# leotimus/recommender-tensorflow

Hardware: AMD Instinct MI355X
Metric: examples/sec DeepFM batch=65536 (full train step) (higher is better)
Workload: dtype f32 (MLP GEMM operands: fp16 hi+lo split, 3 products, fp32 accumulate)

## Files before the change

### __graft_entry__.py

```python
import os
import subprocess
import sys

ROOT = os.path.dirname(os.path.abspath(__file__))
PKG = os.path.join(ROOT, "recommender-tensorflow_amd")
for _p in (ROOT, PKG):
    if _p not in sys.path:
        sys.path.insert(0, _p)


def build():
    csrc = os.path.join(PKG, "csrc")
    subprocess.run(["make", "-C", csrc, "-j", str(min(8, os.cpu_count() or 1))], check=True)
    from mi355x_rec import _lib
    lib = _lib.load()
    print("built:", lib.mi_build_info().decode(), "->", _lib.LIB_PATH)
    import oracle


def smoke():
    import numpy as np
    import torch
    from mi355x_rec.engine import DeepFM, OptimizerSpec
    from oracle import deepfm as O, optimizers as OO
    from oracle.columns import ml100k_fields, sorted_fields

    assert torch.cuda.is_available(), "smoke() needs a GPU"
    cases = (([f[4] for f in sorted_fields(ml100k_fields())], 4, [16, 16], 32),
             ([40 + 3 * i for i in range(26)], 64, [512, 256, 128], 64))
    for vocab, E, hidden, B in cases:
        rng = np.random.default_rng(0)
        p = O.init_params(rng, vocab, E, hidden, dtype=np.float32, lin_scale=0.01)
        m = DeepFM(vocab, embedding_size=E, hidden_units=hidden, optimizer=OptimizerSpec("Adam", 0.001), device="cuda:0")
        m.load_oracle_params(p)
        st = O.TrainState(p, OO.Hyper("Adam", 0.001))
        for _ in range(3):
            ids = np.stack([rng.integers(0, v, B) for v in vocab], 1).astype(np.int32)
            y = (rng.random(B) < 0.3).astype(np.uint8)
            lo, logit_o = O.train_step(p, st, ids, y)
            lg, logit_g = m.train_step(torch.from_numpy(ids).cuda(), torch.from_numpy(y).cuda())
            err = float(np.max(np.abs(logit_g.cpu().numpy() - logit_o)) / (np.sqrt(np.mean(logit_o ** 2)) + 1e-30))
            assert abs(lg.item() - float(lo)) / abs(float(lo)) < 2e-5 and err < 5e-5, (E, lg.item(), float(lo), err)
        print("smoke ok (E=%d, hidden %s, planes path: %s): loss %.6f (oracle %.6f), logits err %.2e" % (
            E, hidden, bool(m.planes), lg.item(), float(lo), err))


if __name__ == "__main__":
    build()
    if "--smoke" in sys.argv:
        smoke()
```

### recommender-tensorflow_amd/csrc/optim.hip

```cpp
#include "common.h"
#include "optim_rules.h"
#include <algorithm>

namespace {

constexpr int kBlock = 256;

__global__ __launch_bounds__(kBlock) void dense_apply_k(float* __restrict__ w, float* __restrict__ s0,
                                                        float* __restrict__ s1,
                                                        const float* __restrict__ g, int64_t n,
                                                        Hp h, const mi_step_state_t* __restrict__ st) {
  if (st) h.lr_t = st->lr_t;
  const int64_t stride = static_cast<int64_t>(gridDim.x) * kBlock;
  for (int64_t i = static_cast<int64_t>(blockIdx.x) * kBlock + threadIdx.x; i < n; i += stride) {
    float wv = w[i], a = s0 ? s0[i] : 0.f, b = s1 ? s1[i] : 0.f;
    dense_rule(h, wv, a, b, g[i]);
    w[i] = wv;
    if (s0) s0[i] = a;
    if (s1) s1[i] = b;
  }
}

typedef float f32x4_t __attribute__((ext_vector_type(4)));
__device__ __forceinline__ float4 ld4_nt(const float* p) {
// ... 198 lines not shown
        if constexpr (STORE) store_row(a, uu, l, lane_on, g, gl);
        else apply_row(a, h, r, l, lane_on, w, g, gl, load_row_state(a, h, r, l, lane_on));
      }
      __syncthreads();
    }
  }
}

__device__ __forceinline__ float sqrt_rn_fixup(float x) {
  float s = __builtin_amdgcn_sqrtf(x);
  const float sm = __uint_as_float(__float_as_uint(s) - 1u), sp = __uint_as_float(__float_as_uint(s) + 1u);
  const float rm = fmaf(-sm, s, x), rp = fmaf(-sp, s, x);
  s = (rm <= 0.f) ? sm : s;
  s = (rp > 0.f) ? sp : s;
  return s;
}
__device__ __forceinline__ float sqrt_rn_inrange(float x) {
  const float r = __builtin_amdgcn_rsqf(x);
  float s = x * r, h = 0.5f * r;
  const float e = fmaf(-h, s, 0.5f);
  h = fmaf(h, e, h);
  s = fmaf(s, e, s);
  const float d = fmaf(-s, s, x);
  return fmaf(d, h, s);
}
__device__ __forceinline__ float div_rn_inrange(float n, float d) {
  float r = __builtin_amdgcn_rcpf(d);
  const float e = fmaf(-d, r, 1.0f);
  r = fmaf(e, r, r);
  float q = n * r;
  const float e2 = fmaf(-d, q, n);
  q = fmaf(e2, r, q);
  const float e3 = fmaf(-d, q, n);
  return fmaf(e3, r, q);
}
__device__ __forceinline__ bool catchup_in_range(float m, float v) {
  const float am = fabsf(m);
  return (am == 0.f || (am >= 0x1p-50f && am <= 0x1p60f)) && v >= 0x1p-93f && v <= 0x1p20f;
}
__device__ __forceinline__ bool catchup_params_in_range(int steps, float lr_last, float eps, float b1, float b2) {
  return steps <= 200 && lr_last >= 0x1p-17f && eps >= 0x1p-40f && eps <= 1.f &&
         b1 >= 0.9f && b1 <= 1.f && b2 >= 0.99f && b2 <= 1.f;
}

struct RhoSplit { float hi, lo; };
__device__ __forceinline__ RhoSplit rho_split(float b2) {
  const double r = sqrt(static_cast<double>(b2));
  RhoSplit q;
  q.hi = static_cast<float>(r);
  q.lo = static_cast<float>(r - static_cast<double>(q.hi));
  return q;
}
__device__ __forceinline__ float bounded_step(float w, float u, float s0, float rj, float eps) {
  return fmaf(-u, __builtin_amdgcn_rcpf(fmaf(s0, rj, eps)), w);
}

__global__ __launch_bounds__(kBlock) void catchup_lin_k(
    float* __restrict__ lin_w, float* __restrict__ lm, float* __restrict__ lv, const int32_t* __restrict__ last_step,
    const int32_t* __restrict__ uniq_rows, const int32_t* __restrict__ num_uniq, int64_t n_max, int step_to,
    const float* __restrict__ lr_table, float b1, float b2, float eps, bool defer_slots, int st,
    const mi_step_state_t* __restrict__ ss, bool bounded) {
  if (ss) step_to = ss->step - 1;
  const int64_t u = static_cast<int64_t>(blockIdx.x) * kBlock + threadIdx.x;
  const int64_t count = uniq_rows ? static_cast<int64_t>(*num_uniq) : n_max;
  const bool on = u < count;
  const int64_t r = (on ? (uniq_rows ? static_cast<int64_t>(uniq_rows[u]) : u) : 0) * st;
  const int ls = on ? last_step[r] : step_to;
  const bool work = on && ls > 0 && ls < step_to;
  float w = 0.f, m = 0.f, v = 0.f;
  if (work) { w = lin_w[r]; m = lm[r]; v = lv[r]; }
  if (bounded) {
    if (work) {
      const RhoSplit rho = rho_split(b2);
      const float s0 = sqrtf(v);
      float rj = 1.f;
      for (int s = ls + 1; s <= step_to; ++s) {
        rj = fmaf(rj, rho.lo, rj * rho.hi);
        m = m * b1;
        w = bounded_step(w, lr_table[s] * m, s0, rj, eps);
      }
      if (!defer_slots)
        for (int s = ls + 1; s <= step_to; ++s) v = v * b2;
      lin_w[r] = w;
      if (!defer_slots) { lm[r] = m; lv[r] = v; }
    }
    return;
  }
  const bool ok = !work || (catchup_params_in_range(step_to - ls, lr_table[step_to], eps, b1, b2) && catchup_in_range(m, v));
  if (__ballot(!ok) == 0) {
    if (work)
      for (int s = ls + 1; s <= step_to; ++s) {
        m = m * b1; v = v * b2;
        w = w - div_rn_inrange(lr_table[s] * m, sqrt_rn_inrange(v) + eps);
      }
  } else if (work) {
    replay(w, m, v, ls + 1, step_to, lr_table, b1, b2, eps);
  }
  if (work) {
    lin_w[r] = w;
    if (!defer_slots) { lm[r] = m; lv[r] = v; }
  }
}

template <int LPR>
__global__ __launch_bounds__(kBlock) void sparse_catchup_k(
    float* __restrict__ table, float* __restrict__ tm, float* __restrict__ tv,
    int32_t* __restrict__ last_step, const int32_t* __restrict__ uniq_rows,
    const int32_t* __restrict__ num_uniq, int64_t n_max, int E, int step_to,
    const float* __restrict__ lr_table, float b1, float b2, float eps, bool defer_slots, int st,
    const mi_step_state_t* __restrict__ ss, bool keep_stamps, int64_t ts) {
  if (ss) step_to = ss->step - 1;
  const int64_t u = (static_cast<int64_t>(blockIdx.x) * kBlock + threadIdx.x) / LPR;
  const int l = threadIdx.x & (LPR - 1);
  const int64_t count = uniq_rows ? static_cast<int64_t>(*num_uniq) : n_max;
  if (u >= count) return;
  const int64_t r = uniq_rows ? static_cast<int64_t>(uniq_rows[u]) : u;
  const int ls = last_step[r * st];
  if (ls >= step_to) return;
  if (ls > 0) {
    if (table && 4 * l < E) {
      const int64_t o = r * ts + 4 * l;
      float4 w = ld4(table + o), m = ld4_nt(tm + o), v = ld4_nt(tv + o);
      const bool ok = catchup_params_in_range(step_to - ls, lr_table[step_to], eps, b1, b2) && catchup_in_range(m.x, v.x) &&
                      catchup_in_range(m.y, v.y) && catchup_in_range(m.z, v.z) && catchup_in_range(m.w, v.w);
      if (__ballot(!ok) == 0) {
        for (int s = ls + 1; s <= step_to; ++s) {
          const float lr = lr_table[s];
          m.x = m.x * b1; m.y = m.y * b1; m.z = m.z * b1; m.w = m.w * b1;
          v.x = v.x * b2; v.y = v.y * b2; v.z = v.z * b2; v.w = v.w * b2;
          w.x = w.x - div_rn_inrange(lr * m.x, sqrt_rn_inrange(v.x) + eps);
          w.y = w.y - div_rn_inrange(lr * m.y, sqrt_rn_inrange(v.y) + eps);
          w.z = w.z - div_rn_inrange(lr * m.z, sqrt_rn_inrange(v.z) + eps);
          w.w = w.w - div_rn_inrange(lr * m.w, sqrt_rn_inrange(v.w) + eps);
        }
      } else
      for (int s = ls + 1; s <= step_to; ++s) {
        const float lr = lr_table[s];
        m.x = m.x * b1; m.y = m.y * b1; m.z = m.z * b1; m.w = m.w * b1;
        v.x = v.x * b2; v.y = v.y * b2; v.z = v.z * b2; v.w = v.w * b2;
        w.x = w.x - (lr * m.x) / (sqrtf(v.x) + eps);
        w.y = w.y - (lr * m.y) / (sqrtf(v.y) + eps);
        w.z = w.z - (lr * m.z) / (sqrtf(v.z) + eps);
        w.w = w.w - (lr * m.w) / (sqrtf(v.w) + eps);
      }
      st4(table + o, w);
      if (!defer_slots) { st4_nt(tm + o, m); st4_nt(tv + o, v); }
    }
  }
  if (l == 0 && !defer_slots && !keep_stamps) last_step[r * st] = step_to;
}

constexpr int kLrWindow = 1024;

struct RowIn { int64_t r; int ls; float4 w, m, v; };

__device__ __forceinline__ RowIn load_row_in(const float* __restrict__ table, const float* __restrict__ tm, const float* __restrict__ tv,
                                             const int32_t* __restrict__ last_step, int64_t r, int64_t ts, int l, bool lane_on, int st) {
  RowIn q;
  q.r = r;
  q.ls = last_step[r * st];
  q.w = q.m = q.v = make_float4(0.f, 0.f, 0.f, 0.f);
  if (lane_on) {
    const int64_t o = r * ts + 4 * l;
    q.w = ld4(table + o); q.m = ld4_nt(tm + o); q.v = ld4_nt(tv + o);
  }
  return q;
}

template <int LPR>
__global__ __launch_bounds__(kBlock) void sparse_catchup_bounded_k(
    float* __restrict__ table, float* __restrict__ tm, float* __restrict__ tv,
    int32_t* __restrict__ last_step, const int32_t* __restrict__ uniq_rows,
    const int32_t* __restrict__ num_uniq, int64_t n_max, int E, int step_to,
    const float* __restrict__ lr_table, float b1, float b2, float eps, bool defer_slots, int st,
    const mi_step_state_t* __restrict__ ss, bool keep_stamps, int64_t ts) {
  __shared__ float lr_s[kLrWindow];
  if (ss) step_to = ss->step - 1;
  const int base = step_to - (kLrWindow - 1);
  for (int i = threadIdx.x; i < kLrWindow; i += kBlock) lr_s[i] = base + i >= 1 ? lr_table[base + i] : 0.f;
  __syncthreads();
  const int l = threadIdx.x & (LPR - 1);
  const bool lane_on = 4 * l < E;
  const int64_t count = uniq_rows ? static_cast<int64_t>(*num_uniq) : n_max;
  constexpr int RPW = 64 / LPR;
  const int64_t n_chunks = (count + RPW - 1) / RPW;
  const int W = static_cast<int>(gridDim.x) * (kBlock / 64);
  const int64_t J = (n_chunks + W - 1) / W;
  const int S = static_cast<int>(J > 0 && W / J > 1 ? W / J : 1);
  const int k = static_cast<int>(blockIdx.x) * (kBlock / 64) + (threadIdx.x >> 6);
  const int grp = (threadIdx.x & 63) / LPR;
  auto row_at = [&](int64_t j) -> int64_t {
    const int64_t seg = (k + j * S) & (W - 1);
    const int64_t c = seg * J + j;
    return c < n_chunks ? c * RPW + grp : count;
  };
  if (J == 0) return;
  const RhoSplit rho = rho_split(b2);
  auto row_id = [&](int64_t x) { return uniq_rows ? uniq_rows[x] : static_cast<int32_t>(x); };
  RowIn none;
  none.r = 0; none.ls = INT32_MAX; none.w = none.m = none.v = make_float4(0.f, 0.f, 0.f, 0.f);
  auto replay = [&](const RowIn& cur) {
    const int ls = cur.ls;
    if (ls > 0 && ls < step_to) {
      if (lane_on) {
        float4 w = cur.w, m = cur.m;
        const float4 s0 = make_float4(fminf(__builtin_amdgcn_sqrtf(cur.v.x), 3.4028234e38f), fminf(__builtin_amdgcn_sqrtf(cur.v.y), 3.4028234e38f),
                                      fminf(__builtin_amdgcn_sqrtf(cur.v.z), 3.4028234e38f), fminf(__builtin_amdgcn_sqrtf(cur.v.w), 3.4028234e38f));
        float rj = 1.f;
        int s = ls + 1;
        for (; s < base && s <= step_to; ++s) {
          const float lr = lr_table[s];
          rj = fmaf(rj, rho.lo, rj * rho.hi);
          m.x = m.x * b1; m.y = m.y * b1; m.z = m.z * b1; m.w = m.w * b1;
          w.x = bounded_step(w.x, lr * m.x, s0.x, rj, eps); w.y = bounded_step(w.y, lr * m.y, s0.y, rj, eps);
          w.z = bounded_step(w.z, lr * m.z, s0.z, rj, eps); w.w = bounded_step(w.w, lr * m.w, s0.w, rj, eps);
        }
        typedef float f32x2 __attribute__((ext_vector_type(2)));
        const f32x2 sa = {s0.x, s0.y}, sb = {s0.z, s0.w};
        const f32x2 ev = {eps, eps}, one = {1.f, 1.f};
        f32x2 ra, rb;
        {
          const f32x2 rv = {rj, rj};
          const f32x2 da = __builtin_elementwise_fma(sa, rv, ev), db = __builtin_elementwise_fma(sb, rv, ev);
          ra.x = __builtin_amdgcn_rcpf(da.x); ra.y = __builtin_amdgcn_rcpf(da.y);
          rb.x = __builtin_amdgcn_rcpf(db.x); rb.y = __builtin_amdgcn_rcpf(db.y);
        }
        f32x2 ma = {m.x, m.y}, mb = {m.z, m.w}, wa = {w.x, w.y}, wb = {w.z, w.w};
#pragma unroll 2
        for (; s <= step_to; ++s) {
          const float lr = lr_s[s - base];
          rj = fmaf(rj, rho.lo, rj * rho.hi);
          ma = ma * b1; mb = mb * b1;
          const f32x2 rv = {rj, rj};
          const f32x2 da = __builtin_elementwise_fma(sa, rv, ev), db = __builtin_elementwise_fma(sb, rv, ev);
          const f32x2 ea = __builtin_elementwise_fma(-da, ra, one), eb = __builtin_elementwise_fma(-db, rb, one);
          const f32x2 pa = __builtin_elementwise_fma(ea, ea, ea), pb = __builtin_elementwise_fma(eb, eb, eb);
          ra = __builtin_elementwise_fma(ra, pa, ra); rb = __builtin_elementwise_fma(rb, pb, rb);
          const f32x2 ua = lr * ma, ub = lr * mb;
          wa = __builtin_elementwise_fma(-ua, ra, wa); wb = __builtin_elementwise_fma(-ub, rb, wb);
        }
        m = make_float4(ma.x, ma.y, mb.x, mb.y); w = make_float4(wa.x, wa.y, wb.x, wb.y);
        const int64_t o = cur.r * ts + 4 * l;
        st4(table + o, w);
        if (!defer_slots) {
          float4 v = cur.v;
          for (int q = ls + 1; q <= step_to; ++q) { v.x = v.x * b2; v.y = v.y * b2; v.z = v.z * b2; v.w = v.w * b2; }
          st4_nt(tm + o, m); st4_nt(tv + o, v);
        }
      }
    }
    if (l == 0 && !defer_slots && !keep_stamps && ls < step_to) last_step[cur.r * st] = step_to;
  };
  int64_t u0 = row_at(0);
  RowIn nxt = u0 < count ? load_row_in(table, tm, tv, last_step, row_id(u0), ts, l, lane_on, st) : none;
  int64_t u1 = J > 1 ? row_at(1) : count;
  int32_t id_pref = u1 < count ? row_id(u1) : 0;
  for (int64_t j = 0; j < J; ++j) {
    const RowIn cur = nxt;
    const int64_t r_next = id_pref;
    const bool more = j + 1 < J;
    if (more) {
      nxt = u1 < count ? load_row_in(table, tm, tv, last_step, r_next, ts, l, lane_on, st) : none;
      u1 = j + 2 < J ? row_at(j + 2) : count;
      if (u1 < count) id_pref = row_id(u1);
    }
    replay(cur);
  }
}

__global__ __launch_bounds__(kBlock) void selftest_sqrt_k(uint32_t first_bits, int64_t count, unsigned long long* __restrict__ mism) {
  const int64_t i = static_cast<int64_t>(blockIdx.x) * kBlock + threadIdx.x;
  bool bad_fast = false, bad_fixup = false;
  if (i < count) {
    const float x = __uint_as_float(first_bits + static_cast<uint32_t>(i));
    const uint32_t ref = __float_as_uint(sqrtf(x));
    bad_fast = __float_as_uint(sqrt_rn_inrange(x)) != ref;
    bad_fixup = __float_as_uint(sqrt_rn_fixup(x)) != ref;
  }
  const unsigned long long bf = __ballot(bad_fast), bx = __ballot(bad_fixup);
  if ((threadIdx.x & 63) == 0) {
    if (bf) atomicAdd(mism, static_cast<unsigned long long>(__popcll(bf)));
    if (bx) atomicAdd(mism + 1, static_cast<unsigned long long>(__popcll(bx)));
  }
}

__global__ __launch_bounds__(kBlock) void gap_keys_k(const int32_t* __restrict__ uniq_rows,
                                                     const int32_t* __restrict__ num_uniq,
                                                     const int32_t* __restrict__ last_step, int64_t n_max, int step_to,
                                                     int32_t* __restrict__ keys, int st,
                                                     const mi_step_state_t* __restrict__ ss) {
  if (ss) step_to = ss->step - 1;
  const int64_t u = static_cast<int64_t>(blockIdx.x) * kBlock + threadIdx.x;
  if (u >= n_max) return;
  int32_t key = 63;
  if (u < *num_uniq) {
    const int ls = last_step[static_cast<int64_t>(uniq_rows[u]) * st];
    key = (ls > 0 && ls < step_to) ? min(step_to - ls, 62) : 0;
  }
  keys[u] = key;
}

int lanes_per_row(int E) {
  int q = (E + 3) / 4, l = 1;
  while (l < q) l <<= 1;
  return l;
}

}

#define MI_DISPATCH_LPR(lpr, CALL)                  \
  switch (lpr) {                                    \
    case 1: { constexpr int L = 1; CALL; } break;   \
    case 2: { constexpr int L = 2; CALL; } break;   \
    case 4: { constexpr int L = 4; CALL; } break;   \
    case 8: { constexpr int L = 8; CALL; } break;   \
    case 16: { constexpr int L = 16; CALL; } break; \
    case 32: { constexpr int L = 32; CALL; } break; \
    default: { constexpr int L = 64; CALL; } break; \
  }

static int32_t check_hp(const char* who, const mi_opt_hparams* hp) {
  if (!hp || hp->kind < MI_OPT_ADAM || hp->kind > MI_OPT_SGD) {
    mi::set_error("%s: bad optimizer kind", who);
    return MI_ERR_INVALID;
  }
  if (hp->kind == MI_OPT_FTRL && hp->lr_power != -0.5f) {
    mi::set_error("%s: Ftrl learning_rate_power %f unsupported (TF default -0.5 only)", who, hp->lr_power);
    return MI_ERR_UNSUPPORTED;
  }
  return MI_OK;
}

__global__ __launch_bounds__(kBlock) void axpy_k(float* __restrict__ y, const float* __restrict__ x, int64_t n, float alpha) {
  const int64_t i = static_cast<int64_t>(blockIdx.x) * kBlock + threadIdx.x;
  if (i < n) y[i] = y[i] + alpha * x[i];
}

unsigned long_grid(int64_t n_max) {
  return static_cast<unsigned>(std::min<int64_t>(1024, mi::ceil_div(n_max, kBlock)));
}

__global__ void step_advance_k(mi_step_state_t* __restrict__ st, const float* __restrict__ lr_table) {
  const int s = st->step + 1;
  st->step = s;
  st->lr_t = lr_table ? lr_table[s] : 0.f;
  st->seed_term = static_cast<uint64_t>(s) * 1000003ull;
}

extern "C" {

int32_t mi_step_advance(mi_step_state_t* device_state, const float* lr_table, mi_stream_t stream) {
  MI_REQUIRE(device_state, "step_advance: null state");
  step_advance_k<<<dim3(1), dim3(1), 0, mi::as_stream(stream)>>>(device_state, lr_table);
  MI_CHECK_LAUNCH("step_advance");
  return MI_OK;
}

int32_t mi_axpy(float* y, const float* x, int64_t n, float alpha, mi_stream_t stream) {
  MI_REQUIRE(n >= 0 && (n == 0 || (x && y)), "axpy: n=%lld", (long long)n);
  if (n == 0) return MI_OK;
  axpy_k<<<dim3((unsigned)mi::ceil_div(n, kBlock)), dim3(kBlock), 0, mi::as_stream(stream)>>>(y, x, n, alpha);
  MI_CHECK_LAUNCH("axpy");
  return MI_OK;
}


int32_t mi_dense_apply(float* param, float* slot0, float* slot1, const float* grad, int64_t n,
                       const mi_opt_hparams* hp, mi_stream_t stream) {
  if (int32_t rc = check_hp("dense_apply", hp)) return rc;
  MI_REQUIRE(n >= 0, "dense_apply: n=%lld", (long long)n);
  if (n == 0) return MI_OK;
  MI_REQUIRE(param && grad, "dense_apply: null buffer");
  MI_REQUIRE(hp->kind == MI_OPT_SGD || slot0, "dense_apply: optimizer needs slot0");
  MI_REQUIRE((hp->kind != MI_OPT_ADAM && hp->kind != MI_OPT_FTRL && hp->kind != MI_OPT_RMSPROP) || slot1,
             "dense_apply: optimizer needs slot1");
  int64_t nb = mi::ceil_div(n, kBlock);
  if (nb > 4096) nb = 4096;
  dense_apply_k<<<dim3((unsigned)nb), dim3(kBlock), 0, mi::as_stream(stream)>>>(param, slot0, slot1, grad, n, make_hp(hp), mi::step_state());
  MI_CHECK_LAUNCH("dense_apply");
  return MI_OK;
}

int32_t mi_sparse_apply(float* table, float* t_slot0, float* t_slot1, float* lin_w, float* l_slot0,
                        float* l_slot1, int32_t* last_step, const int32_t* uniq_rows,
                        const int32_t* seg_start, const int32_t* sorted_entry,
                        const int32_t* num_uniq, int64_t n_max, const float* d_rows,
                        const float* d_lin, int32_t E, int32_t step, const mi_opt_hparams* hp,
                        int32_t lin_stride, int64_t table_stride, int64_t grad_stride, mi_stream_t stream) {
  if (int32_t rc = check_hp("sparse_apply", hp)) return rc;
  MI_REQUIRE(grad_stride == 0 || (grad_stride >= (table ? E : 1) && (!table || (grad_stride & 3) == 0)),
             "sparse_apply: grad_stride=%lld (0 = d_rows E apart and d_lin 1 apart, else one record per entry)", (long long)grad_stride);
  if (!table) table_stride = 0;
  MI_REQUIRE(table_stride == 0 || (table_stride >= E && (table_stride & 3) == 0), "%s: table_stride=%lld (0 = E, else >= E and a multiple of 4)", "sparse_apply", (long long)table_stride);
  const int64_t ts = table_stride ? table_stride : E;

  MI_REQUIRE(lin_stride >= 1, "sparse_apply: lin_stride=%d", lin_stride);
  MI_REQUIRE(n_max >= 0, "sparse_apply: n_max=%lld", (long long)n_max);
  if (n_max == 0) return MI_OK;
  MI_REQUIRE(table || lin_w, "sparse_apply: nothing to update");
  MI_REQUIRE(uniq_rows && seg_start && sorted_entry && num_uniq, "sparse_apply: null index buffer");
  MI_REQUIRE(!table || (d_rows && E >= 4 && E <= 256 && (E & 3) == 0 && mi::aligned16(table) && mi::aligned16(d_rows)),
             "sparse_apply: table needs d_rows, E multiple of 4 in [4,256], 16-byte alignment");
  MI_REQUIRE(!lin_w || d_lin, "sparse_apply: lin_w needs d_lin");
  const bool need0 = hp->kind != MI_OPT_SGD;
  const bool need1 = hp->kind == MI_OPT_ADAM || hp->kind == MI_OPT_FTRL || hp->kind == MI_OPT_RMSPROP;
  MI_REQUIRE(!table || ((!need0 || t_slot0) && (!need1 || t_slot1)), "sparse_apply: table slots missing");
  MI_REQUIRE(!lin_w || ((!need0 || l_slot0) && (!need1 || l_slot1)), "sparse_apply: linear slots missing");
  const int lpr = table ? lanes_per_row(E) : 1;
  const int64_t blocks = mi::ceil_div(n_max * lpr, kBlock);
  MI_REQUIRE(blocks <= INT32_MAX, "sparse_apply: grid too large");
  const Hp h = make_hp(hp);
  ApplyArgs a{table, t_slot0, t_slot1, lin_w, l_slot0, l_slot1, last_step, uniq_rows, seg_start, sorted_entry,
              num_uniq, d_rows, d_lin, E, step};
  a.ls = lin_stride; a.ts = ts;
  a.gs = grad_stride ? grad_stride : E; a.gls = grad_stride ? grad_stride : 1;
  a.st = mi::step_state();
  MI_DISPATCH_LPR(lpr, (sparse_apply_k<L, false><<<dim3((unsigned)blocks), dim3(kBlock), 0, mi::as_stream(stream)>>>(
                           a, h, FusedGrad{})));
  MI_CHECK_LAUNCH("sparse_apply");
  if (n_max > kLongSeg) {
    MI_DISPATCH_LPR(lpr, (sparse_apply_long_k<L, false><<<dim3(long_grid(n_max)), dim3(kBlock), 0, mi::as_stream(stream)>>>(
                             a, h, FusedGrad{})));
    MI_CHECK_LAUNCH("sparse_apply(long segments)");
  }
  return MI_OK;
}

int32_t mi_sparse_apply_fused(float* table, float* t_slot0, float* t_slot1, float* lin_w, float* l_slot0,
                              float* l_slot1, int32_t* last_step, const int32_t* uniq_rows,
                              const int32_t* seg_start, const int32_t* sorted_entry, const int32_t* num_uniq,
                              int64_t n_max, const float* d_concat, int64_t ld_dconcat, const float* sumv,
                              const float* d_logit_fm, const float* d_logit_lin, int32_t F, int32_t E,
                              int32_t step, const mi_opt_hparams* hp, int32_t lin_stride, int64_t table_stride, mi_stream_t stream) {
  if (int32_t rc = check_hp("sparse_apply_fused", hp)) return rc;
  if (!table) table_stride = 0;
  MI_REQUIRE(table_stride == 0 || (table_stride >= E && (table_stride & 3) == 0), "%s: table_stride=%lld (0 = E, else >= E and a multiple of 4)", "sparse_apply_fused", (long long)table_stride);
  const int64_t ts = table_stride ? table_stride : E;

  MI_REQUIRE(lin_stride >= 1, "sparse_apply_fused: lin_stride=%d", lin_stride);
  MI_REQUIRE(n_max >= 0 && F > 0, "sparse_apply_fused: n_max=%lld F=%d", (long long)n_max, F);
  if (n_max == 0) return MI_OK;
  MI_REQUIRE(table || lin_w, "sparse_apply_fused: nothing to update");
  MI_REQUIRE(uniq_rows && seg_start && sorted_entry && num_uniq, "sparse_apply_fused: null index buffer");
  MI_REQUIRE(!table || (E >= 4 && E <= 256 && (E & 3) == 0 && mi::aligned16(table)),
             "sparse_apply_fused: E multiple of 4 in [4,256], 16-byte alignment");
  MI_REQUIRE(!table || d_concat || d_logit_fm, "sparse_apply_fused: table update needs d_concat and/or d_logit_fm");
  MI_REQUIRE(!d_concat || (ld_dconcat >= (int64_t)F * E && (ld_dconcat & 3) == 0 && mi::aligned16(d_concat)),
             "sparse_apply_fused: d_concat leading dimension / alignment");
  MI_REQUIRE(!d_logit_fm || (sumv ? mi::aligned16(sumv) : d_concat != nullptr),
             "sparse_apply_fused: FM gradient needs sumv, or a d_concat that already carries d_logit_fm * sumv");
  MI_REQUIRE(!lin_w || d_logit_lin, "sparse_apply_fused: lin_w needs d_logit_lin");
  const bool need0 = hp->kind != MI_OPT_SGD;
  const bool need1 = hp->kind == MI_OPT_ADAM || hp->kind == MI_OPT_FTRL || hp->kind == MI_OPT_RMSPROP;
  MI_REQUIRE(!table || ((!need0 || t_slot0) && (!need1 || t_slot1)), "sparse_apply_fused: table slots missing");
  MI_REQUIRE(!lin_w || ((!need0 || l_slot0) && (!need1 || l_slot1)), "sparse_apply_fused: linear slots missing");
  const int lpr = table ? lanes_per_row(E) : 1;
  const int64_t blocks = mi::ceil_div(n_max * lpr, kBlock);
  MI_REQUIRE(blocks <= INT32_MAX, "sparse_apply_fused: grid too large");
  const Hp h = make_hp(hp);
  const FusedGrad fg{d_concat, ld_dconcat, sumv, d_logit_fm, d_logit_lin, F, 0};
  ApplyArgs a{table, t_slot0, t_slot1, lin_w, l_slot0, l_slot1, last_step, uniq_rows, seg_start, sorted_entry,
              num_uniq, nullptr, nullptr, E, step};
  a.ls = lin_stride; a.ts = ts;
  a.st = mi::step_state();
  MI_DISPATCH_LPR(lpr, (sparse_apply_k<L, true><<<dim3((unsigned)blocks), dim3(kBlock), 0, mi::as_stream(stream)>>>(a, h, fg)));
  MI_CHECK_LAUNCH("sparse_apply_fused");
  if (n_max > kLongSeg) {
    MI_DISPATCH_LPR(lpr, (sparse_apply_long_k<L, true><<<dim3(long_grid(n_max)), dim3(kBlock), 0, mi::as_stream(stream)>>>(a, h, fg)));
    MI_CHECK_LAUNCH("sparse_apply_fused(long segments)");
  }
  return MI_OK;
}

int32_t mi_entry_grads_segsum(const float* rows, const int32_t* seg_start, const int32_t* sorted_entry, int64_t u_begin,
                              int64_t u_count, const float* d_concat, int64_t ld_dconcat, const float* sumv,
                              const float* d_logit_fm, const float* d_logit_lin, int64_t b0, int32_t F, int32_t E,
                              float* out_rows, float* out_lin, int64_t out_row0, int64_t rows_stride, int64_t out_stride,
                              mi_stream_t stream) {
  MI_REQUIRE(rows_stride == 0 || (rows_stride >= E && (rows_stride & 3) == 0), "entry_grads_segsum: rows_stride=%lld", (long long)rows_stride);
  MI_REQUIRE(out_stride == 0 || (out_stride >= (out_rows ? E : 1) && (!out_rows || (out_stride & 3) == 0)),
             "entry_grads_segsum: out_stride=%lld (0 = out_rows E apart and out_lin 1 apart, else one record per request)", (long long)out_stride);
  MI_REQUIRE(u_begin >= 0 && u_count >= 0 && u_begin + u_count <= INT32_MAX && F > 0 && b0 >= 0, "entry_grads_segsum: u_begin=%lld u_count=%lld",
             (long long)u_begin, (long long)u_count);
  MI_REQUIRE(out_row0 >= 0 && out_row0 <= u_begin, "entry_grads_segsum: out_row0=%lld must lie in [0, u_begin=%lld]", (long long)out_row0,
             (long long)u_begin);
  if (u_count == 0) return MI_OK;
  MI_REQUIRE(seg_start && sorted_entry && (out_rows || out_lin), "entry_grads_segsum: null buffer");
  MI_REQUIRE(!out_rows || (E >= 4 && E <= 256 && (E & 3) == 0 && mi::aligned16(out_rows) && (d_concat || d_logit_fm)),
             "entry_grads_segsum: row gradients need E multiple of 4 in [4,256] and d_concat and/or d_logit_fm");
  MI_REQUIRE(!d_concat || (ld_dconcat >= (int64_t)F * E && (ld_dconcat & 3) == 0 && mi::aligned16(d_concat)),
             "entry_grads_segsum: d_concat leading dimension / alignment");
  MI_REQUIRE(!d_logit_fm || (sumv && rows && mi::aligned16(sumv) && mi::aligned16(rows)), "entry_grads_segsum: the FM gradient needs sumv and the rows");
  MI_REQUIRE(!out_lin || d_logit_lin, "entry_grads_segsum: out_lin needs d_logit_lin");
  const int lpr = out_rows ? lanes_per_row(E) : 1;
  const int64_t blocks = mi::ceil_div(u_count * lpr, kBlock);
  MI_REQUIRE(blocks <= INT32_MAX, "entry_grads_segsum: grid too large");
  const FusedGrad fg{d_concat, ld_dconcat, sumv, d_logit_fm, d_logit_lin, F, b0};
  ApplyArgs a{};
  a.table = out_rows ? const_cast<float*>(rows) : nullptr;
  if (out_rows && !rows) a.table = out_rows;
  a.lin_w = out_lin;
  a.seg_start = seg_start; a.sorted_entry = sorted_entry;
  a.E = E;
  a.os = out_stride ? out_stride : E; a.ols = out_stride ? out_stride : 1;
  a.out_rows = out_rows ? reinterpret_cast<float*>(reinterpret_cast<uintptr_t>(out_rows) - static_cast<uintptr_t>(out_row0) * a.os * sizeof(float)) : nullptr;
  a.out_lin = out_lin ? reinterpret_cast<float*>(reinterpret_cast<uintptr_t>(out_lin) - static_cast<uintptr_t>(out_row0) * a.ols * sizeof(float)) : nullptr;
  a.u_begin = (int)u_begin; a.u_count = (int)u_count; a.ls = 1;
  a.ts = rows_stride ? rows_stride : E;
  const Hp h{};
  MI_DISPATCH_LPR(lpr, (sparse_apply_k<L, true, true><<<dim3((unsigned)blocks), dim3(kBlock), 0, mi::as_stream(stream)>>>(a, h, fg)));
  MI_CHECK_LAUNCH("entry_grads_segsum");
  if (u_count > 0) {
    MI_DISPATCH_LPR(lpr, (sparse_apply_long_k<L, true, true><<<dim3(long_grid(u_count)), dim3(kBlock), 0, mi::as_stream(stream)>>>(a, h, fg)));
    MI_CHECK_LAUNCH("entry_grads_segsum(long segments)");
  }
  return MI_OK;
}

int32_t mi_selftest_sqrt(uint32_t first_bits, int64_t count, uint64_t* mismatches, mi_stream_t stream) {
  MI_REQUIRE(count >= 0 && static_cast<uint64_t>(first_bits) + static_cast<uint64_t>(count) <= (1ull << 32), "selftest_sqrt: range leaves 32 bits");
  if (count == 0) return MI_OK;
  MI_REQUIRE(mismatches, "selftest_sqrt: null buffer");
  const int64_t blocks = mi::ceil_div(count, kBlock);
  MI_REQUIRE(blocks <= INT32_MAX, "selftest_sqrt: grid too large");
  selftest_sqrt_k<<<dim3((unsigned)blocks), dim3(kBlock), 0, mi::as_stream(stream)>>>(
      first_bits, count, reinterpret_cast<unsigned long long*>(mismatches));
  MI_CHECK_LAUNCH("selftest_sqrt");
  return MI_OK;
}

int32_t mi_catchup_gap_keys(const int32_t* uniq_rows, const int32_t* num_uniq, const int32_t* last_step, int64_t n_max,
                            int32_t step_to, int32_t* keys, int32_t lin_stride, mi_stream_t stream) {
  MI_REQUIRE(n_max >= 0 && step_to >= 0 && lin_stride >= 1, "catchup_gap_keys: n_max=%lld", (long long)n_max);
  if (n_max == 0) return MI_OK;
  MI_REQUIRE(uniq_rows && num_uniq && last_step && keys, "catchup_gap_keys: null buffer");
  gap_keys_k<<<dim3((unsigned)mi::ceil_div(n_max, kBlock)), dim3(kBlock), 0, mi::as_stream(stream)>>>(
      uniq_rows, num_uniq, last_step, n_max, step_to, keys, lin_stride, mi::step_state());
  MI_CHECK_LAUNCH("catchup_gap_keys");
  return MI_OK;
}

int32_t mi_sparse_catchup(float* table, float* t_m, float* t_v, float* lin_w, float* l_m, float* l_v,
                          int32_t* last_step, const int32_t* uniq_rows, const int32_t* num_uniq,
                          int64_t n_max, int32_t E, int32_t step_to, const float* lr_table,
                          float beta1, float beta2, float epsilon, int32_t flags, int32_t lin_stride,
                          int64_t table_stride, mi_stream_t stream) {
  MI_REQUIRE(n_max >= 0 && step_to >= 0 && lin_stride >= 1, "sparse_catchup: n_max=%lld step_to=%d", (long long)n_max, step_to);
  if (!table) table_stride = 0;
  MI_REQUIRE(table_stride == 0 || (table_stride >= E && (table_stride & 3) == 0), "%s: table_stride=%lld (0 = E, else >= E and a multiple of 4)", "sparse_catchup", (long long)table_stride);
  const int64_t ts = table_stride ? table_stride : E;

  MI_REQUIRE((flags & ~(MI_CATCHUP_DEFER_SLOTS | MI_CATCHUP_BOUNDED | MI_CATCHUP_KEEP_STAMPS)) == 0, "sparse_catchup: flags=%d", flags);
  const bool keep_stamps = (flags & MI_CATCHUP_KEEP_STAMPS) != 0;
  const int32_t defer_slots = flags & MI_CATCHUP_DEFER_SLOTS;
  const bool bounded = (flags & MI_CATCHUP_BOUNDED) != 0 && epsilon >= 1e-30f && beta2 > 0.f && beta2 <= 1.f;
  if (n_max == 0 || (step_to == 0 && !mi::step_state())) return MI_OK;
  MI_REQUIRE(last_step && lr_table, "sparse_catchup: null buffer");
  MI_REQUIRE(table || lin_w, "sparse_catchup: nothing to update");
  MI_REQUIRE(!table || (t_m && t_v && E >= 4 && E <= 256 && (E & 3) == 0 && mi::aligned16(table)),
             "sparse_catchup: table needs m, v, E multiple of 4 in [4,256]");
  MI_REQUIRE(!lin_w || (l_m && l_v), "sparse_catchup: lin_w needs m, v");
  MI_REQUIRE(!uniq_rows || num_uniq, "sparse_catchup: uniq_rows without num_uniq");
  const bool defer = defer_slots != 0 && uniq_rows != nullptr;
  if (lin_w) {
    catchup_lin_k<<<dim3((unsigned)mi::ceil_div(n_max, kBlock)), dim3(kBlock), 0, mi::as_stream(stream)>>>(
        lin_w, l_m, l_v, last_step, uniq_rows, num_uniq, n_max, step_to, lr_table, beta1, beta2, epsilon, defer, lin_stride, mi::step_state(),
        bounded);
    MI_CHECK_LAUNCH("sparse_catchup(wide part)");
  }
  if (!table && (defer || keep_stamps)) return MI_OK;
  const int lpr = table ? lanes_per_row(E) : 1;
  const int64_t blocks = mi::ceil_div(n_max * lpr, kBlock);
  MI_REQUIRE(blocks <= INT32_MAX, "sparse_catchup: grid too large");
  if (bounded && table) {
    int64_t pb = mi::env_int("MI_CATCHUP_BLOCKS", 1024);
    while (pb > 1 && pb > blocks) pb >>= 1;
    MI_DISPATCH_LPR(lpr, (sparse_catchup_bounded_k<L><<<dim3((unsigned)pb), dim3(kBlock), 0, mi::as_stream(stream)>>>(
                             table, t_m, t_v, last_step, uniq_rows, num_uniq, n_max, E, step_to, lr_table, beta1, beta2,
                             epsilon, defer, lin_stride, mi::step_state(), keep_stamps, ts)));
  } else {
    MI_DISPATCH_LPR(lpr, (sparse_catchup_k<L><<<dim3((unsigned)blocks), dim3(kBlock), 0, mi::as_stream(stream)>>>(
                             table, t_m, t_v, last_step, uniq_rows, num_uniq, n_max, E, step_to, lr_table, beta1, beta2,
                             epsilon, defer, lin_stride, mi::step_state(), keep_stamps, ts)));
  }
  MI_CHECK_LAUNCH("sparse_catchup");
  return MI_OK;
}

}
```

### recommender-tensorflow_amd/mi355x_rec/engine.py

```python
import ctypes as C
import json
import os
import math

import numpy as np
import torch

from . import _lib
from ._lib import OptHparams, check, ptr

OPT_KINDS = {"Adam": 0, "Adagrad": 1, "Ftrl": 2, "RMSProp": 3, "SGD": 4}


def _align(n, a=16):
    return (n + a - 1) // a * a


class HipKernels:

    supports_planes = True

    def __init__(self):
        self.lib = _lib.load()
        self.timers = None
# ... 1014 lines not shown

    def top_k(self, query_ids, candidate_ids, query_fields, k, query_x=None, candidate_x=None, exclude=None,
              return_scores=False):
        if self.shard is not None:
            raise NotImplementedError("top_k runs on one GPU: a row-sharded engine has only its shard of the tables")
        nf = self.F + self.n_numeric
        qf = [int(f) for f in query_fields]
        if len(set(qf)) != len(qf) or any(f < 0 or f >= nf for f in qf):
            raise ValueError("query_fields %r must be distinct column indices in [0, %d)" % (list(query_fields), nf))
        cf = [f for f in range(nf) if f not in set(qf)]
        if not qf or not cf:
            raise ValueError("query_fields must split the %d columns into two non-empty sides" % nf)
        k = int(k)
        if not 1 <= k <= self.TOP_K_MAX:
            raise ValueError("k=%d outside [1, %d]" % (k, self.TOP_K_MAX))
        sides = []
        for name, fields, ids, x in (("query", qf, query_ids, query_x), ("candidate", cf, candidate_ids, candidate_x)):
            cat = sorted(f for f in fields if f < self.F)
            num = sorted(f - self.F for f in fields if f >= self.F)
            if not isinstance(ids, torch.Tensor) or ids.dtype != torch.int32 or ids.dim() != 2 or ids.shape[1] != len(cat) \
                    or not ids.is_contiguous() or ids.device.type != self.device.type:
                raise ValueError("%s_ids must be a contiguous int32 [n, %d] tensor on %s" % (name, len(cat), self.device))
            n = ids.shape[0]
            if n < 1:
                raise ValueError("%s_ids: no rows" % name)
            if num:
                if not isinstance(x, torch.Tensor) or x.dtype != torch.float32 or tuple(x.shape) != (n, len(num)) \
                        or not x.is_contiguous() or x.device.type != self.device.type:
                    raise ValueError("%s_x must be a contiguous float32 [%d, %d] tensor on %s" % (name, n, len(num), self.device))
            elif x is not None:
                raise ValueError("%s_x given but the %s side has no numeric column" % (name, name))
            sides.append((cat, num, ids, x, n))
        U, I = sides[0][4], sides[1][4]
        excl_off = excl_idx = None
        if exclude is not None:
            if isinstance(exclude, tuple) and len(exclude) == 2:
                off = np.asarray(exclude[0].cpu() if isinstance(exclude[0], torch.Tensor) else exclude[0], np.int64)
                idx = np.asarray(exclude[1].cpu() if isinstance(exclude[1], torch.Tensor) else exclude[1], np.int32)
            else:
                rows = [np.asarray(sorted(set(int(c) for c in r)), np.int32) for r in exclude]
                if len(rows) != U:
                    raise ValueError("exclude: %d rows for %d queries" % (len(rows), U))
                off = np.concatenate([[0], np.cumsum([len(r) for r in rows])]).astype(np.int64)
                idx = np.concatenate(rows + [np.zeros(0, np.int32)]).astype(np.int32)
            if off.shape != (U + 1,) or off[0] != 0 or np.any(np.diff(off) < 0) or off[-1] != idx.size:
                raise ValueError("exclude: offsets must be a non-decreasing [U + 1] array from 0 to len(indices)")
            if idx.size and (idx.min() < 0 or idx.max() >= I):
                raise ValueError("exclude: candidate index outside [0, %d)" % I)
            excl_off = torch.from_numpy(off).to(self.device)
            excl_idx = torch.from_numpy(np.ascontiguousarray(idx) if idx.size else np.zeros(1, np.int32)).to(self.device)
        self.finalize_rows()
        k_ = self.k
        k_.query("mi_set_gemm_mode", 0)
        (a_q, s_q, w_q), (a_c, s_c, w_c) = [self._side_tensors(*s[:4], candidate=i == 1) for i, s in enumerate(sides)]
        H1 = self.layers[0][3] if self.use_dnn else 0
        rest = self.layers[1:] if self.use_dnn else []
        layer_off = torch.tensor([o for (ko, bo, _, _) in rest for o in (ko, bo)] or [0], dtype=torch.int64)
        widths = torch.tensor([H1] + [h for (_, _, _, h) in rest], dtype=torch.int32)
        E = self.E if self.use_mf else 0
        top_score = torch.empty(U, k, dtype=torch.float32, device=self.device)
        top_idx = torch.empty(U, k, dtype=torch.int32, device=self.device)
        scores = torch.empty(U, I, dtype=torch.float32, device=self.device) if return_scores else None
        ws = self._bytes("topk_ws", k_.query("mi_pair_topk_workspace_bytes", U, I, k, H1, E))
        k_.mi_pair_topk(a_q, s_q, w_q, U, a_c, s_c, w_c, I, H1, E, self.dense, layer_off, widths, len(rest), self.act,
                        excl_off, excl_idx, k, top_score, top_idx, scores, ws, ws.numel())
        return (top_score, top_idx, scores) if return_scores else (top_score, top_idx)

    def _side_tensors(self, cat, num, ids, x, candidate):
        k = self.k
        dev, E, n = self.device, self.E, ids.shape[0]
        f32 = dict(dtype=torch.float32, device=dev)
        Fx, nx = len(cat), len(num)
        raw = self.raw_numeric
        emb_num = 0 if raw else nx
        d_emb = (Fx + emb_num) * E if self.use_emb else 0
        D = _align(d_emb + (nx if (raw and self.use_dnn) else 0), 4)
        concat = torch.zeros(n, max(D, 4), **f32) if (self.use_dnn or (nx and not raw and self.use_emb)) else None
        sumv = torch.zeros(n, E, **f32) if self.use_mf else None
        fm = torch.zeros(n, **f32) if self.use_mf else None
        lin = torch.zeros(n, **f32) if self.use_linear else None
        field_off = self.field_off[cat].contiguous() if Fx else None
        if Fx and self.use_emb and (concat is not None or sumv is not None):
            k.mi_embed_fm_linear_fwd(self.table, None, field_off, ids, n, Fx, E, concat, concat.shape[1] if concat is not None
                                     else 0, sumv, fm, None, None, 1, self.ts)
        if Fx and lin is not None:
            wide = [j for j, f in enumerate(cat) if self.wide_fields is None or self.wide_fields[f]]
            if wide:
                w_ids = ids if len(wide) == Fx else ids[:, wide].contiguous()
                k.mi_embed_fm_linear_fwd(None, self.lin_w, self.field_off[[cat[j] for j in wide]].contiguous(), w_ids, n,
                                         len(wide), E, None, 0, None, None, lin, None, self.ls, 0)
        if nx:
            jj = torch.tensor(num, dtype=torch.int64, device=dev)
            wn = self._seg(self.dense, self.lin_num_off, (self.n_numeric,))[jj].contiguous() if self.use_linear else None
            if raw:
                if concat is not None or lin is not None:
                    k.mi_numeric_raw_fwd(x, wn, n, nx, concat if self.use_dnn else None, D, d_emb, D - d_emb, lin)
            else:
                V = self._seg(self.dense, self.num_emb_off, (self.n_numeric, E))[jj].contiguous()
                k.mi_numeric_embed_fwd(x, V, wn, n, nx, E, concat, concat.shape[1], Fx * E, sumv, fm, lin)
        a = None
        if self.use_dnn:
            H1 = self.layers[0][3]
            rows = [f * E + j for f in cat for j in range(E)] if self.use_emb else []
            if raw:
                rows += [self.D_emb + j for j in num]
            else:
                rows += [self.F * E + j * E + e for j in num for e in range(E)]
            a = torch.empty(n, H1, **f32)
            b0 = self.bias(0) if candidate else torch.zeros(H1, **f32)
            if rows:
                W = torch.zeros(D, H1, **f32)
                W[:len(rows)] = self.kernel(0)[torch.tensor(rows, dtype=torch.int64, device=dev)]
                k.mi_dense_fwd(concat, concat.shape[1], W, b0, a, H1, n, H1, D, 0, 1.0, 0, None)
            else:
                a.copy_(b0.expand(n, H1))
        w = None
        if lin is not None or fm is not None:
            w = torch.empty(n, **f32)
            lb = self.dense[self.lin_bias_off:] if (candidate and self.use_linear) else None
            hws = self._bytes("topk_head_ws", k.query("mi_head_workspace_bytes", n))
            k.mi_sigmoid_ce_head(lin, lb, fm, None, None, n, 1.0, w, None, None, None, hws, hws.numel())
        elif candidate and self.use_linear:
            w = self.dense[self.lin_bias_off:self.lin_bias_off + 1].expand(n).contiguous()
        return a, sumv, w

    GAP_SORT_MIN = 16384
    TOP_FUSED_MIN_BATCH = 4096
    GRAPH_SHAPES_MAX = 4

    def _new_side_stream(self, priority=0):
        n = self.__dict__.setdefault("_n_side", {})
        k = n[priority] = n.get(priority, -1) + 1
        return _tested_side_stream(self.device, priority, k)

    def _catchup(self, uniq, num_uniq, n_max, defer=False, by_gap=None):
        t_adam = self.opt.name == "Adam" and self.table is not None
        l_adam = (self.lin_opt or self.opt).name == "Adam" and self.lin_w is not None
        if not (t_adam or l_adam) or n_max == 0:
            return
        defer = bool(defer and uniq is not None and self.lin_opt is None)
        for sc in (self.sched, self.lin_sched):
            if sc is not None:
                sc.lr_t(self.step)
        if uniq is not None and n_max >= self.GAP_SORT_MIN:
            uniq = by_gap if by_gap is not None else self._rows_by_gap(uniq, num_uniq, n_max, self.step)
        flags = (1 if defer else 0) | (2 if self.catchup == "bounded" else 0)
        t_sched = self.sched if t_adam else None
        l_sched = (self.lin_sched if self.lin_opt is not None else (self.lin_sched or self.sched)) if l_adam else None
        side = None
        if t_sched is not None and l_sched is not None and t_sched is not l_sched:
            assert not defer
            parts = [(None, l_sched, 4), (t_sched, None, 0)]
        elif (defer and t_sched is not None and l_sched is not None and self.shard is None and self.device.type == "cuda"
              and self._wide_on_side_stream(n_max // max(self.F, 1))):
            parts = [(None, l_sched, 0), (t_sched, None, 0)]
            side = self._side_stream()
            side.wait_stream(torch.cuda.current_stream())
        else:
            parts = [(t_sched, l_sched, 0)]
        for i, (ts, lsch, extra) in enumerate(parts):
            s = (ts or lsch).spec
            entry = self.k.tagged("mi_sparse_catchup", "/wide") if (ts is None and hasattr(self.k, "tagged")) else self.k.mi_sparse_catchup
            call = lambda entry=entry: entry(
                self.table if ts is not None else None, self.t_s0 if ts is not None else None,
                self.t_s1 if ts is not None else None, self.lin_w if lsch is not None else None,
                self.l_s0 if lsch is not None else None, self.l_s1 if lsch is not None else None,
                self.last_step, uniq, num_uniq, n_max, self.E, self.step, (ts or lsch).table, s.beta1, s.beta2,
                s.epsilon, flags | extra, self.ls, self.ts)
            if side is not None and i == 0:
                with torch.cuda.stream(side):
                    call()
            else:
                call()

    def _side_stream(self):
        side = self._ws.get("side_stream")
        if side is None:
            side = self._ws["side_stream"] = self._new_side_stream()
        return side

    def _wide_on_side_stream(self, B):
        return (self.device.type == "cuda" and self.use_emb and self.use_linear and self.use_dnn and self.n_numeric == 0
                and self.F > 0 and B >= 4096)

    def _sort_unique(self, keys, n, key_range, tag, ws_name="sort_ws", cap=None, slot=None):
        i32 = torch.int32
        cap = max(n, cap or 0)
        sorted_entry = self._buf(tag + "_sorted", (cap,), i32)[:n]
        uniq = self._buf(tag + "_uniq", (cap,), i32)[:n]
        seg = self._buf(tag + "_seg", (cap + 1,), i32)[:n + 1]
        num_uniq = self._buf(tag + "_nu", (1,), i32)
        ws = self._bytes(ws_name, self.k.query("mi_sort_unique_workspace_bytes", cap))
        if slot is not None:
            self.k.mi_sort_unique_rows_slots(keys, n, key_range, sorted_entry, uniq, seg, num_uniq, slot, ws, ws.numel())
        else:
            self.k.mi_sort_unique_rows(keys, n, key_range, sorted_entry, uniq, seg, num_uniq, ws, ws.numel())
        return sorted_entry, uniq, seg, num_uniq

    PRESORT_MIN = 16384

    def _sort_batch(self, ids, tag, side=False):
        k = self.k
        B = ids.shape[0]
        n = B * self.F
        if B % 4096 == 0 and self.F <= 64 and hasattr(k, "mi_sort_unique_fields"):
            i32 = torch.int32
            sorted_entry, uniq = self._buf(tag + "_sorted", (n,), i32), self._buf(tag + "_uniq", (n,), i32)
            seg, num_uniq = self._buf(tag + "_seg", (n + 1,), i32), self._buf(tag + "_nu", (1,), i32)
            ws = self._bytes("sortf_ws", k.query("mi_sort_unique_fields_workspace_bytes", B, self.F))
            sort = k.tagged("mi_sort_unique_fields", "/next batch, side stream") if (side and hasattr(k, "tagged")) else k.mi_sort_unique_fields
            sort(ids, self.field_off, B, self.F, self.max_vocab, sorted_entry, uniq, seg, num_uniq, ws, ws.numel(), 1 if side else 0)
            return sorted_entry, uniq, seg, num_uniq
        rows = self._buf("rows", (n,), torch.int32)
        k.mi_global_rows(ids, self.field_off, B, self.F, rows)
        return self._sort_unique(rows, n, self.R, tag)

    def _presort(self, next_ids, tag):
        side = self._ws.get("presort_stream")
        if side is None:
            side = self._ws["presort_stream"] = self._new_side_stream()
        main = torch.cuda.current_stream()
        side.wait_stream(main)
        with torch.cuda.stream(side):
            out = self._sort_batch(next_ids, tag, side=True)
        self._presorted = {"ids": next_ids, "version": next_ids._version, "tag": tag, "sorted": out, "stream": side,
                           "by_gap": None, "by_gap_step": None}

    def _by_gap_ahead(self):
        ps = self._presorted
        if ps is None or not self.adam_rows:
            return
        n = ps["ids"].shape[0] * self.F
        if n < self.GAP_SORT_MIN:
            return
        side = ps["stream"]
        side.wait_stream(torch.cuda.current_stream())
        with torch.cuda.stream(side):
            ps["by_gap"] = self._rows_by_gap(ps["sorted"][1], ps["sorted"][3], n, self.step + 1, ps["tag"] + "_ahead", side=True)
        ps["by_gap_step"] = self.step + 1

    def _rows_by_gap(self, uniq, num_uniq, n_max, step_to, tag="", side=False):
        by_gap = self._buf("uniq_by_gap" + tag, (n_max,), torch.int32)
        ws = self._bytes("gap_ws" + tag, self.k.query("mi_sort_unique_workspace_bytes", n_max))
        f = self.k.tagged("mi_catchup_rows_by_gap", "/next batch, side stream") if (side and hasattr(self.k, "tagged")) else \
            self.k.mi_catchup_rows_by_gap
        f(uniq, num_uniq, self.last_step, n_max, step_to, self.ls, by_gap, ws, ws.numel())
        return by_gap

    def train_step(self, ids, labels, x_num=None, next_ids=None):
        self._prep(ids, labels, x_num)
        if self.shard is not None:
            from . import parallel
            return parallel.sharded_train_step(self, ids, labels, x_num, next_ids)
        return self._train_step_single(ids, labels, x_num, next_ids)

    def _take_presorted(self, ids):
        ps, self._presorted = getattr(self, "_presorted", None), None
        if ps is None:
            return None
        torch.cuda.current_stream().wait_stream(ps["stream"])
        if ps["ids"].data_ptr() == ids.data_ptr() and ps["ids"].shape == ids.shape and ps["version"] == ids._version:
            return ps
        return None

    def _announce(self, ids, next_ids, x_num, tag):
        B = ids.shape[0]
        if (next_ids is not None and self.device.type == "cuda" and B * self.F >= self.PRESORT_MIN and next_ids.shape == ids.shape
                and B % 4096 == 0 and self.F <= 64 and hasattr(self.k, "mi_sort_unique_fields")
                and not getattr(self, "_capturing", False)):
            self._prep(next_ids, None, x_num)
            self._presort(next_ids, "own2" if tag == "own" else "own")

    def _train_step_single(self, ids, labels, x_num, next_ids):
        B = ids.shape[0]
        n = B * self.F
        if n == 0:
            c = self._forward(ids, x_num, True)
            logits, loss, dlogit = self._head(c, labels, True)
            self._backward_dense(c, dlogit)
            self._apply(None, None, None, None, 0, None, None)
            return loss, logits
        self._split_weights_ahead()
        ps = self._take_presorted(ids)
        tag = ps["tag"] if ps is not None else "own"
        sorted_entry, uniq, seg, num_uniq = ps["sorted"] if ps is not None else self._sort_batch(ids, tag)
        self._announce(ids, next_ids, x_num, tag)
        if self.adam_rows and self.step > 0:
            by_gap = ps["by_gap"] if (ps is not None and ps.get("by_gap_step") == self.step) else None
            self._catchup(uniq, num_uniq, n, defer=True, by_gap=by_gap)
        c = self._forward(ids, x_num, True)
        logits, loss, dlogit = self._head(c, labels, True)
        self._by_gap_ahead()
        d_concat = self._backward_dense(c, dlogit)
        self._apply(uniq, seg, sorted_entry, num_uniq, n, None, None, fused=(d_concat, c["sumv"], dlogit))
        return loss, logits

    def _entry_grads(self, c, d_concat, dlogit, pos, d_rows=None, d_lin=None):
        B = c["B"]
        n = B * self.F
        if d_rows is None and self.use_emb:
            d_rows = self._buf("d_rows", (n, self.E))
        if d_lin is None and self.use_linear:
            d_lin = self._buf("d_lin", (n,))
        rows = c["g_table"] if (c["concat"] is None and self.use_mf) else None
        self.k.mi_embed_fm_linear_bwd(d_concat, self.D, c["concat"], self.D, rows, c["sumv"],
                                      dlogit if self.use_mf else None, dlogit if self.use_linear else None, pos,
                                      B, self.F, self.E, d_rows, d_lin)
# ... 350 lines not shown
```

Baseline: 24.19 million.

## Fuse wide linear-term Adam catchup into bounded embedding catchup kernel

When the linear weights are stored as packed 4-float records (w, m, v, last_step), the bounded sparse catch-up kernel now replays the linear-term Adam update alongside the embedding row. This drops the separate catchup_lin_k launch and the side-stream split, and reads the step stamp from the packed record. The fused variant also gets a waves-per-EU hint. The trade-off is extra per-row work and registers in the hot kernel. The build step also gains a 'tuning' make target.

```diff
diff --git a/__graft_entry__.py b/__graft_entry__.py
--- a/__graft_entry__.py
+++ b/__graft_entry__.py
@@ -12,6 +12,7 @@
 def build():
     csrc = os.path.join(PKG, "csrc")
     subprocess.run(["make", "-C", csrc, "-j", str(min(8, os.cpu_count() or 1))], check=True)
+    subprocess.run(["make", "-C", csrc, "tuning", "-j", str(min(8, os.cpu_count() or 1))], check=True)
     from mi355x_rec import _lib
     lib = _lib.load()
     print("built:", lib.mi_build_info().decode(), "->", _lib.LIB_PATH)
diff --git a/recommender-tensorflow_amd/csrc/optim.hip b/recommender-tensorflow_amd/csrc/optim.hip
--- a/recommender-tensorflow_amd/csrc/optim.hip
+++ b/recommender-tensorflow_amd/csrc/optim.hip
@@ -374,13 +374,21 @@
 
 constexpr int kLrWindow = 1024;
 
-struct RowIn { int64_t r; int ls; float4 w, m, v; };
-
+struct RowIn { int64_t r; int ls; float4 w, m, v; float lw, lm, lv; };
+
+template <bool WIDE>
 __device__ __forceinline__ RowIn load_row_in(const float* __restrict__ table, const float* __restrict__ tm, const float* __restrict__ tv,
-                                             const int32_t* __restrict__ last_step, int64_t r, int64_t ts, int l, bool lane_on, int st) {
+                                             const int32_t* __restrict__ last_step, const float* lin_w, int64_t r, int64_t ts, int l,
+                                             bool lane_on, int st) {
   RowIn q;
   q.r = r;
-  q.ls = last_step[r * st];
+  q.lw = q.lm = q.lv = 0.f;
+  if constexpr (WIDE) {
+    const float4 rec = ld4(lin_w + r * 4);
+    q.lw = rec.x; q.lm = rec.y; q.lv = rec.z; q.ls = __float_as_int(rec.w);
+  } else {
+    q.ls = last_step[r * st];
+  }
   q.w = q.m = q.v = make_float4(0.f, 0.f, 0.f, 0.f);
   if (lane_on) {
     const int64_t o = r * ts + 4 * l;
@@ -389,10 +397,10 @@
   return q;
 }
 
-template <int LPR>
-__global__ __launch_bounds__(kBlock) void sparse_catchup_bounded_k(
+template <int LPR, bool WIDE>
+__global__ __launch_bounds__(kBlock) __attribute__((amdgpu_waves_per_eu(WIDE ? 7 : 1))) void sparse_catchup_bounded_k(
     float* __restrict__ table, float* __restrict__ tm, float* __restrict__ tv,
-    int32_t* __restrict__ last_step, const int32_t* __restrict__ uniq_rows,
+    int32_t* __restrict__ last_step, float* lin_w, const int32_t* __restrict__ uniq_rows,
     const int32_t* __restrict__ num_uniq, int64_t n_max, int E, int step_to,
     const float* __restrict__ lr_table, float b1, float b2, float eps, bool defer_slots, int st,
     const mi_step_state_t* __restrict__ ss, bool keep_stamps, int64_t ts) {
@@ -421,6 +429,7 @@
   auto row_id = [&](int64_t x) { return uniq_rows ? uniq_rows[x] : static_cast<int32_t>(x); };
   RowIn none;
   none.r = 0; none.ls = INT32_MAX; none.w = none.m = none.v = make_float4(0.f, 0.f, 0.f, 0.f);
+  none.lw = none.lm = none.lv = 0.f;
   auto replay = [&](const RowIn& cur) {
     const int ls = cur.ls;
     if (ls > 0 && ls < step_to) {
@@ -428,11 +437,14 @@
         float4 w = cur.w, m = cur.m;
         const float4 s0 = make_float4(fminf(__builtin_amdgcn_sqrtf(cur.v.x), 3.4028234e38f), fminf(__builtin_amdgcn_sqrtf(cur.v.y), 3.4028234e38f),
                                       fminf(__builtin_amdgcn_sqrtf(cur.v.z), 3.4028234e38f), fminf(__builtin_amdgcn_sqrtf(cur.v.w), 3.4028234e38f));
+        float lw = cur.lw, lm = cur.lm;
+        const float ls0 = WIDE ? sqrtf(cur.lv) : 0.f;
         float rj = 1.f;
         int s = ls + 1;
         for (; s < base && s <= step_to; ++s) {
           const float lr = lr_table[s];
           rj = fmaf(rj, rho.lo, rj * rho.hi);
+          if constexpr (WIDE) { lm = lm * b1; lw = bounded_step(lw, lr * lm, ls0, rj, eps); }
           m.x = m.x * b1; m.y = m.y * b1; m.z = m.z * b1; m.w = m.w * b1;
           w.x = bounded_step(w.x, lr * m.x, s0.x, rj, eps); w.y = bounded_step(w.y, lr * m.y, s0.y, rj, eps);
           w.z = bounded_step(w.z, lr * m.z, s0.z, rj, eps); w.w = bounded_step(w.w, lr * m.w, s0.w, rj, eps);
@@ -452,6 +464,7 @@
         for (; s <= step_to; ++s) {
           const float lr = lr_s[s - base];
           rj = fmaf(rj, rho.lo, rj * rho.hi);
+          if constexpr (WIDE) { lm = lm * b1; lw = bounded_step(lw, lr * lm, ls0, rj, eps); }
           ma = ma * b1; mb = mb * b1;
           const f32x2 rv = {rj, rj};
           const f32x2 da = __builtin_elementwise_fma(sa, rv, ev), db = __builtin_elementwise_fma(sb, rv, ev);
@@ -464,17 +477,31 @@
         m = make_float4(ma.x, ma.y, mb.x, mb.y); w = make_float4(wa.x, wa.y, wb.x, wb.y);
         const int64_t o = cur.r * ts + 4 * l;
         st4(table + o, w);
+        float lv = cur.lv;
         if (!defer_slots) {
           float4 v = cur.v;
-          for (int q = ls + 1; q <= step_to; ++q) { v.x = v.x * b2; v.y = v.y * b2; v.z = v.z * b2; v.w = v.w * b2; }
+          for (int q = ls + 1; q <= step_to; ++q) {
+            v.x = v.x * b2; v.y = v.y * b2; v.z = v.z * b2; v.w = v.w * b2;
+            if constexpr (WIDE) lv = lv * b2;
+          }
           st4_nt(tm + o, m); st4_nt(tv + o, v);
         }
+        if constexpr (WIDE) {
+          if (l == 0) {
+            float* rec = lin_w + cur.r * 4;
+            rec[0] = lw;
+            if (!defer_slots) { rec[1] = lm; rec[2] = lv; }
+          }
+        }
       }
     }
-    if (l == 0 && !defer_slots && !keep_stamps && ls < step_to) last_step[cur.r * st] = step_to;
+    if (l == 0 && !defer_slots && !keep_stamps && ls < step_to) {
+      if constexpr (WIDE) lin_w[cur.r * 4 + 3] = __int_as_float(step_to);
+      else last_step[cur.r * st] = step_to;
+    }
   };
   int64_t u0 = row_at(0);
-  RowIn nxt = u0 < count ? load_row_in(table, tm, tv, last_step, row_id(u0), ts, l, lane_on, st) : none;
+  RowIn nxt = u0 < count ? load_row_in<WIDE>(table, tm, tv, last_step, lin_w, row_id(u0), ts, l, lane_on, st) : none;
   int64_t u1 = J > 1 ? row_at(1) : count;
   int32_t id_pref = u1 < count ? row_id(u1) : 0;
   for (int64_t j = 0; j < J; ++j) {
@@ -482,7 +509,7 @@
     const int64_t r_next = id_pref;
     const bool more = j + 1 < J;
     if (more) {
-      nxt = u1 < count ? load_row_in(table, tm, tv, last_step, r_next, ts, l, lane_on, st) : none;
+      nxt = u1 < count ? load_row_in<WIDE>(table, tm, tv, last_step, lin_w, r_next, ts, l, lane_on, st) : none;
       u1 = j + 2 < J ? row_at(j + 2) : count;
       if (u1 < count) id_pref = row_id(u1);
     }
@@ -784,7 +811,10 @@
   MI_REQUIRE(!lin_w || (l_m && l_v), "sparse_catchup: lin_w needs m, v");
   MI_REQUIRE(!uniq_rows || num_uniq, "sparse_catchup: uniq_rows without num_uniq");
   const bool defer = defer_slots != 0 && uniq_rows != nullptr;
-  if (lin_w) {
+  const bool wide_fused = table && lin_w && bounded && lin_stride == 4 && l_m == lin_w + 1 && l_v == lin_w + 2 &&
+                          reinterpret_cast<float*>(last_step) == lin_w + 3 && mi::aligned16(lin_w) &&
+                          mi::env_int("MI_CATCHUP_WIDE", 1) != 0;
+  if (lin_w && !wide_fused) {
     catchup_lin_k<<<dim3((unsigned)mi::ceil_div(n_max, kBlock)), dim3(kBlock), 0, mi::as_stream(stream)>>>(
         lin_w, l_m, l_v, last_step, uniq_rows, num_uniq, n_max, step_to, lr_table, beta1, beta2, epsilon, defer, lin_stride, mi::step_state(),
         bounded);
@@ -797,9 +827,15 @@
   if (bounded && table) {
     int64_t pb = mi::env_int("MI_CATCHUP_BLOCKS", 1024);
     while (pb > 1 && pb > blocks) pb >>= 1;
-    MI_DISPATCH_LPR(lpr, (sparse_catchup_bounded_k<L><<<dim3((unsigned)pb), dim3(kBlock), 0, mi::as_stream(stream)>>>(
-                             table, t_m, t_v, last_step, uniq_rows, num_uniq, n_max, E, step_to, lr_table, beta1, beta2,
-                             epsilon, defer, lin_stride, mi::step_state(), keep_stamps, ts)));
+    if (wide_fused) {
+      MI_DISPATCH_LPR(lpr, (sparse_catchup_bounded_k<L, true><<<dim3((unsigned)pb), dim3(kBlock), 0, mi::as_stream(stream)>>>(
+                               table, t_m, t_v, last_step, lin_w, uniq_rows, num_uniq, n_max, E, step_to, lr_table, beta1, beta2,
+                               epsilon, defer, lin_stride, mi::step_state(), keep_stamps, ts)));
+    } else {
+      MI_DISPATCH_LPR(lpr, (sparse_catchup_bounded_k<L, false><<<dim3((unsigned)pb), dim3(kBlock), 0, mi::as_stream(stream)>>>(
+                               table, t_m, t_v, last_step, nullptr, uniq_rows, num_uniq, n_max, E, step_to, lr_table, beta1, beta2,
+                               epsilon, defer, lin_stride, mi::step_state(), keep_stamps, ts)));
+    }
   } else {
     MI_DISPATCH_LPR(lpr, (sparse_catchup_k<L><<<dim3((unsigned)blocks), dim3(kBlock), 0, mi::as_stream(stream)>>>(
                              table, t_m, t_v, last_step, uniq_rows, num_uniq, n_max, E, step_to, lr_table, beta1, beta2,
diff --git a/recommender-tensorflow_amd/mi355x_rec/engine.py b/recommender-tensorflow_amd/mi355x_rec/engine.py
--- a/recommender-tensorflow_amd/mi355x_rec/engine.py
+++ b/recommender-tensorflow_amd/mi355x_rec/engine.py
@@ -1190,7 +1190,7 @@
             assert not defer
             parts = [(None, l_sched, 4), (t_sched, None, 0)]
         elif (defer and t_sched is not None and l_sched is not None and self.shard is None and self.device.type == "cuda"
-              and self._wide_on_side_stream(n_max // max(self.F, 1))):
+              and self._wide_on_side_stream(n_max // max(self.F, 1)) and not (self.catchup == "bounded" and self.ls == 4)):
             parts = [(None, l_sched, 0), (t_sched, None, 0)]
             side = self._side_stream()
             side.wait_stream(torch.cuda.current_stream())
```

Result: slower. 23.90 million (-1.2%).
